# facebookresearch/mbrl-lib

Measured on AMD Instinct MI355X. Metric: candidate-steps/sec (pop×particles×horizon / plan) per CEM iter; plans/sec, higher is better.
Workload: dtype f32

## Files before the change

### mbrl-lib_amd/csrc/cem.hpp

```cpp
#pragma once
#include <type_traits>

#include "common.hpp"

namespace hipets {

struct CemDev {
    int n_env;
    int pop, H, A, D;
    int K;
    float alpha, one_minus_alpha;
    int return_mean, clipped, unbiased;
    const float* totals = nullptr;
    int P = 0;
    const int* elite_in = nullptr;
};

__device__ __forceinline__ float philox_trunc_normal(uint32_t idx_lo, uint32_t idx_hi, uint64_t seed, uint64_t stream) {
    for (uint32_t attempt = 0; attempt < 64; ++attempt) {
        const Philox4 r = philox4x32_10(idx_lo, idx_hi, attempt, (uint32_t)stream, (uint32_t)seed,
                                        (uint32_t)(seed >> 32) ^ (uint32_t)(stream >> 32) ^ 0x5EED5EEDu);
        float n0, n1, n2, n3;
        box_muller(r.x, r.y, n0, n1);
        if (fabsf(n0) <= 2.0f) return n0;
        if (fabsf(n1) <= 2.0f) return n1;
        box_muller(r.z, r.w, n2, n3);
        if (fabsf(n2) <= 2.0f) return n2;
        if (fabsf(n3) <= 2.0f) return n3;
    }
    return 0.0f;
}

__device__ __forceinline__ float philox_normal(uint32_t idx_lo, uint32_t idx_hi, uint64_t seed, uint64_t stream) {
    const Philox4 r = philox4x32_10(idx_lo, idx_hi, 0u, (uint32_t)stream, (uint32_t)seed,
                                    (uint32_t)(seed >> 32) ^ (uint32_t)(stream >> 32) ^ 0x5EED5EEDu);
    float n0, n1;
    box_muller(r.x, r.y, n0, n1);
    return n0;
}

__global__ void cem_sample_kernel(const CemDev p, const float* __restrict__ mu, const float* __restrict__ disp,
                                  const float* __restrict__ lower, const float* __restrict__ upper,
                                  const float* __restrict__ z_in, unsigned long long seed, unsigned long long stream,
                                  float* __restrict__ population) {
    const long long i = (long long)blockIdx.x * blockDim.x + threadIdx.x;
    if (i >= (long long)p.n_env * p.pop * p.D) return;
    const int d = (int)(i % p.D);
    const int env = (int)(i / ((long long)p.pop * p.D));
    const float m = mu[env * p.D + d], v = disp[env * p.D + d], lb = lower[d], ub = upper[d];
    float x;
    if (p.clipped) {
        const float z = z_in ? z_in[i] : philox_normal((uint32_t)i, (uint32_t)(i >> 32), seed, stream);
        x = m + v * z;
        x = x > lb ? x : lb;
        x = x < ub ? x : ub;
    } else {
        const float lbd = (m - lb) / 2.0f, ubd = (ub - m) / 2.0f;
        const float mv = fminf(lbd * lbd, ubd * ubd);
        const float cv = fminf(mv, v);
        const float z = z_in ? z_in[i] : philox_trunc_normal((uint32_t)i, (uint32_t)(i >> 32), seed, stream);
        x = z * sqrtf(cv) + m;
    }
    population[i] = x;
}

#ifndef HIPETS_REFIT_SKIP
#define HIPETS_REFIT_SKIP 0
#endif
constexpr int kRefitThreads = 1024;
constexpr int kMaxPop = 8192;
constexpr int kRefitScratchBytes = 12288;
constexpr int kSelectMaxK = 1024;
constexpr int kRankSortMax = 640;

__global__ __launch_bounds__(kRefitThreads) void cem_refit_kernel(const CemDev p, float* values, const float* population, float* mu,
                                                                 float* disp, float* best_value, float* best_solution,
                                                                 int* elite_idx_out) {
    extern __shared__ __attribute__((aligned(16))) char smem[];
    {
        const int env = blockIdx.y;
        values += (size_t)env * p.pop;
        if (p.totals && !(HIPETS_REFIT_SKIP & 1)) {
            const float* tot = p.totals + (size_t)env * p.pop * p.P;
            for (int i = threadIdx.x; i < p.pop; i += kRefitThreads) {
                float s = 0.f;
                for (int q0 = 0; q0 < p.P; q0 += 8) {
                    float tv[8];
#pragma unroll
                    for (int u = 0; u < 8; ++u) tv[u] = tot[(size_t)i * p.P + min(q0 + u, p.P - 1)];
#pragma unroll
                    for (int u = 0; u < 8; ++u)
                        if (q0 + u < p.P) s += tv[u];
                }
                values[i] = s / (float)p.P;
            }
        }
        population += (size_t)env * p.pop * p.D;
        mu += (size_t)env * p.D;
        disp += (size_t)env * p.D;
        best_value += env;
        best_solution += (size_t)env * p.D;
        if (elite_idx_out) elite_idx_out += (size_t)env * p.K;
    }
    const int* const elite_in = p.elite_in ? p.elite_in + (size_t)blockIdx.y * p.K : nullptr;
    int n2 = 1;
    while (n2 < p.pop) n2 <<= 1;
    float* key = reinterpret_cast<float*>(smem);
    int* idx = reinterpret_cast<int*>(smem + (size_t)n2 * 4);
    const int tid = threadIdx.x;
    for (int i = tid; i < n2; i += kRefitThreads) {
        float v = -INFINITY;
        if (i < p.pop) {
            v = values[i];
            if (v != v) { v = -1e-10f; values[i] = v; }
        }
        key[i] = v;
        idx[i] = i < p.pop ? i : 0x7FFFFFFF;
    }
    __syncthreads();
    if (elite_in) {
        auto in_range = [&](const int e) { return e < 0 ? 0 : (e >= p.pop ? p.pop - 1 : e); };
        const float top_key = key[in_range(elite_in[0])];
        __syncthreads();
        for (int k = tid; k < p.K; k += kRefitThreads) idx[k] = in_range(elite_in[k]);
        if (tid == 0) key[0] = top_key;
        __syncthreads();
    } else if (HIPETS_REFIT_SKIP & 2) {
    } else if (p.pop <= kRankSortMax) {
        for (int i = tid; i < p.pop; i += kRefitThreads) {
            const float ki = key[i];
            int rank = 0;
#pragma unroll 8
            for (int j = 0; j < i; ++j) rank += key[j] >= ki;
#pragma unroll 8
            for (int j = i + 1; j < p.pop; ++j) rank += key[j] > ki;
            idx[i] = rank;
        }
        __syncthreads();
        int* pos = reinterpret_cast<int*>(smem + (size_t)n2 * 8);
        for (int i = tid; i < p.pop; i += kRefitThreads) pos[idx[i]] = i;
        __syncthreads();
        float top_key = key[pos[0]];
        __syncthreads();
        for (int i = tid; i < p.pop; i += kRefitThreads) idx[i] = pos[i];
        if (tid == 0) key[0] = top_key;
        __syncthreads();
    } else if (p.K <= kSelectMaxK) {
        int* hist = reinterpret_cast<int*>(smem + (size_t)n2 * 8);
        int* ctl = hist + 256;
        int* elist = ctl + 8;
        float* ekey = reinterpret_cast<float*>(elist + kSelectMaxK);
        auto okey = [](float v) {
            const unsigned u = __float_as_uint(v + 0.0f);
            return (u & 0x80000000u) ? ~u : (u | 0x80000000u);
        };
        if (tid == 0) { ctl[0] = 0; ctl[1] = 0; ctl[2] = p.K; ctl[3] = 0; }
        for (int pass = 3; pass >= 0; --pass) {
            for (int b = tid; b < 256; b += kRefitThreads) hist[b] = 0;
            __syncthreads();
            const unsigned prefix = (unsigned)ctl[0], mask = (unsigned)ctl[1];
            for (int i = tid; i < p.pop; i += kRefitThreads) {
                const unsigned u = okey(key[i]);
                if ((u & mask) == prefix) atomicAdd(&hist[(u >> (8 * pass)) & 255u], 1);
            }
            __syncthreads();
            if (tid < 64) {
                const int h0 = hist[4 * tid], h1 = hist[4 * tid + 1], h2 = hist[4 * tid + 2], h3 = hist[4 * tid + 3];
                const int mine = h0 + h1 + h2 + h3;
                int above = mine;
#pragma unroll
                for (int d = 1; d < 64; d <<= 1) {
                    const int o = __shfl_down(above, d, 64);
                    if (tid + d < 64) above += o;
                }
                const int need = ctl[2];
                const int higher = above - mine;
                if (higher < need && need <= above) {
// ... 31 lines not shown
        if (tid < p.K) {
            my_id = elist[tid];
            my_key = ekey[tid];
            int rank = 0;
            for (int f = 0; f < p.K; ++f) {
                const float kf = ekey[f];
                rank += (kf > my_key) || (kf == my_key && elist[f] < my_id);
            }
            my_pos = rank;
        }
        __syncthreads();
        if (my_pos >= 0) idx[my_pos] = my_id;
        if (my_pos == 0) key[0] = my_key;
        __syncthreads();
    } else
    for (int k = 2; k <= n2; k <<= 1) {
        for (int j = k >> 1; j > 0; j >>= 1) {
            for (int i = tid; i < n2; i += kRefitThreads) {
                const int ixj = i ^ j;
                if (ixj > i) {
                    const float ka = key[i], kb = key[ixj];
                    const int ia = idx[i], ib = idx[ixj];
                    const bool a_first = (ka > kb) || (ka == kb && ia < ib);
                    const bool up = (i & k) == 0;
                    if (up ? !a_first : a_first) {
                        key[i] = kb; key[ixj] = ka;
                        idx[i] = ib; idx[ixj] = ia;
                    }
                }
            }
            __syncthreads();
        }
    }
    if (elite_idx_out && blockIdx.x == 0)
        for (int k = tid; k < p.K; k += kRefitThreads) elite_idx_out[k] = idx[k];

    const float top = key[0];
    const bool improved = blockIdx.x == 0 && top > best_value[0];
    const int top_i = idx[0];
    __syncthreads();

    double* red = reinterpret_cast<double*>(smem + (size_t)n2 * 8);
    const int nb = (int)gridDim.x, bx = (int)blockIdx.x;
    const int Dslice = (((p.D + nb - 1) / nb + 63) / 64) * 64;
    const int d_lo = bx * Dslice, d_hi = min(p.D, d_lo + Dslice);
    int parts = kRefitThreads / Dslice;
    parts = parts < 1 ? 1 : (parts > 8 ? 8 : parts);
    const int G = kRefitThreads / parts;
    const int part = tid / G, dloc = tid % G;
    const int nu = (p.K + parts - 1) / parts;
    auto sweep = [&](const int base, auto nu_tag, auto hold_tag) __attribute__((always_inline)) {
        constexpr int NU = decltype(nu_tag)::value;
        constexpr bool HOLD = decltype(hold_tag)::value;
        const int d = base + dloc;
        const bool live = d < d_hi && part < parts;
        float mu_old = 0.f, disp_old = 0.f;
        float xv[NU];
        double s = 0.0;
        if (live) {
            if (part == 0) { mu_old = mu[d]; disp_old = disp[d]; }
            for (int k0 = part; k0 < (HOLD ? part + 1 : p.K); k0 += parts * NU) {
#pragma unroll
                for (int u = 0; u < NU; ++u) xv[u] = population[(size_t)idx[min(k0 + u * parts, p.K - 1)] * p.D + d];
#pragma unroll
                for (int u = 0; u < NU; ++u)
                    if (k0 + u * parts < p.K) s += (double)xv[u];
            }
        }
        red[tid] = s;
        __syncthreads();
        double mean = 0.0;
        if (live) {
            for (int q = 0; q < parts; ++q) mean += red[q * G + dloc];
            mean /= (double)p.K;
        }
        __syncthreads();
        double ss = 0.0;
        if (live) {
            for (int k0 = part; k0 < (HOLD ? part + 1 : p.K); k0 += parts * NU) {
                if constexpr (!HOLD) {
#pragma unroll
                    for (int u = 0; u < NU; ++u) xv[u] = population[(size_t)idx[min(k0 + u * parts, p.K - 1)] * p.D + d];
                }
#pragma unroll
                for (int u = 0; u < NU; ++u)
                    if (k0 + u * parts < p.K) {
                        const double dv = (double)xv[u] - mean;
                        ss += dv * dv;
                    }
            }
        }
        red[tid] = ss;
        __syncthreads();
        if (live && part == 0) {
            double var = 0.0;
            for (int q = 0; q < parts; ++q) var += red[q * G + dloc];
            var /= (double)(p.unbiased ? (p.K - 1) : p.K);
            const float new_mu = (float)mean;
            const float new_disp = p.clipped ? (float)sqrt(var) : (float)var;
            mu[d] = p.alpha * mu_old + p.one_minus_alpha * new_mu;
            disp[d] = p.alpha * disp_old + p.one_minus_alpha * new_disp;
        }
        __syncthreads();
    };
    constexpr int kBestHold = 4;
    float best_row[kBestHold];
    const bool best_held = p.D <= kBestHold * kRefitThreads;
    if (improved && best_held) {
#pragma unroll
        for (int u = 0; u < kBestHold; ++u) best_row[u] = population[(size_t)top_i * p.D + min(tid + u * kRefitThreads, p.D - 1)];
    }
    for (int base = d_lo; base < ((HIPETS_REFIT_SKIP & 4) ? d_lo : d_hi); base += G) {
        using T = std::true_type;
        using F = std::false_type;
        if (nu <= 2) sweep(base, std::integral_constant<int, 2>{}, T{});
        else if (nu <= 4) sweep(base, std::integral_constant<int, 4>{}, T{});
        else if (nu <= 8) sweep(base, std::integral_constant<int, 8>{}, T{});
        else if (nu <= 16) sweep(base, std::integral_constant<int, 16>{}, T{});
        else sweep(base, std::integral_constant<int, 16>{}, F{});
    }
    if (improved) {
        if (best_held) {
#pragma unroll
            for (int u = 0; u < kBestHold; ++u)
                if (tid + u * kRefitThreads < p.D) best_solution[tid + u * kRefitThreads] = best_row[u];
        } else {
            for (int d = tid; d < p.D; d += kRefitThreads) best_solution[d] = population[(size_t)top_i * p.D + d];
        }
        if (tid == 0) best_value[0] = top;
    }
}

inline int refit_blocks(const int D) { return D <= 128 ? 1 : (D + 127) / 128 > 8 ? 8 : (D + 127) / 128; }

__global__ void cem_init_kernel(const CemDev p, const float* x0, const float* lower, const float* upper, float* mu,
                                float* disp, float* best_value) {
    const int i = blockIdx.x * blockDim.x + threadIdx.x;
    if (i < p.n_env * p.D) {
        const int d = i % p.D;
        mu[i] = x0[i];
        const float w = upper[d] - lower[d];
        disp[i] = p.clipped ? 1.0f : (w * w) / 16.0f;
    }
    if (i < p.n_env) best_value[i] = -INFINITY;
}

}
```

### mbrl-lib_amd/csrc/engine.hip

```cpp
#include <cstdarg>
#include <cstdio>
#include <cstring>

#include "engine.hpp"

namespace hipets {

thread_local std::string g_err;
thread_local int g_err_kind = HIPETS_ERR_NONE;

int fail(const char* fmt, ...) {
    char buf[1024];
    va_list ap;
    va_start(ap, fmt);
    vsnprintf(buf, sizeof(buf), fmt, ap);
    va_end(ap);
    g_err = buf;
    g_err_kind = HIPETS_ERR_INVALID_ARGUMENT;
    return 1;
}

int fail_kind(const int kind, const char* fmt, ...) {
    char buf[1024];
    va_list ap;
// ... 51 lines not shown

int hipets_create(int device, hipets_engine** out) {
    if (!out) return fail("null out pointer");
    *out = nullptr;
    int n = 0;
    hipError_t err = hipGetDeviceCount(&n);
    if (err != hipSuccess || n <= 0)
        return fail("no HIP device visible (%s) -- libhipets has no CPU fallback", hipGetErrorString(err));
    if (device < 0 || device >= n) return fail("device %d out of range (%d visible)", device, n);
    HCHECK(hipSetDevice(device));
    hipDeviceProp_t prop;
    HCHECK(hipGetDeviceProperties(&prop, device));
    if (std::string(prop.gcnArchName).rfind("gfx950", 0) != 0)
        return fail("device %d is %s; libhipets is built for gfx950 (MI355X) only", device, prop.gcnArchName);
    auto* e = new hipets_engine();
    e->device = device;
    e->num_cu = prop.multiProcessorCount > 0 ? prop.multiProcessorCount : 256;
    e->lds_max = prop.sharedMemPerBlockOptin > 0 ? (size_t)prop.sharedMemPerBlockOptin : (size_t)prop.sharedMemPerBlock;
    if (e->lds_max > 160 * 1024) e->lds_max = 160 * 1024;
    if (hipHostMalloc(reinterpret_cast<void**>(&e->error_flag), sizeof(int), hipHostMallocMapped) != hipSuccess) e->error_flag = nullptr;
    if (e->error_flag) *e->error_flag = 0;
    const char* np = std::getenv("HIPETS_NO_PERSISTENT");
    e->persistent_ok = e->error_flag != nullptr && !(np && np[0] == '1');
    if (e->census.ensure(2 * sizeof(int))) e->persistent_ok = false;
    *out = e;
    return 0;
}

void hipets_destroy(hipets_engine* e) {
    if (!e) return;
    (void)hipSetDevice(e->device);
    comm_release(e);
    for (DevBuf* b : {&e->w3pack, &e->wpack, &e->bpack, &e->layer_meta, &e->norm_mean, &e->norm_std, &e->min_lv, &e->max_lv, &e->no_delta, &e->members,
                      &e->s0, &e->state, &e->totals, &e->term, &e->exchange, &e->step_keys, &e->plan_keys, &e->mu, &e->disp, &e->population, &e->values,
                      &e->best_value, &e->best_solution, &e->past_action, &e->kept, &e->elite_idx, &e->keep_idx, &e->planet_w, &e->planet_b, &e->planet_member, &e->planet_ops, &e->shard_values, &e->gathered, &e->census, &e->train_slab, &e->train_partial})
        b->release();
    for (auto& ev : e->events) { (void)hipEventDestroy(ev.first); (void)hipEventDestroy(ev.second); }
    for (auto& ev : e->event_pool) { (void)hipEventDestroy(ev.first); (void)hipEventDestroy(ev.second); }
    if (e->error_flag) (void)hipHostFree(e->error_flag);
    if (e->last_done) (void)hipEventDestroy(e->last_done);
    for (auto& sl : e->stage) {
        if (sl.p) (void)hipHostFree(sl.p);
        if (sl.done) (void)hipEventDestroy(sl.done);
    }
    delete e;
}

int hipets_set_plan_mode(hipets_engine* e, int32_t mode) {
    if (!e) return fail("null engine");
    if (mode != HIPETS_MODE_FAST && mode != HIPETS_MODE_DEVICE) return fail("plan mode must be HIPETS_MODE_FAST or HIPETS_MODE_DEVICE");
    e->plan_mode = mode;
    return 0;
}

int hipets_set_persistent(hipets_engine* e, int32_t on) {
    if (!e) return fail("null engine");
    if (on && !e->error_flag) return fail("persistent DEVICE-mode launches need the host-mapped timeout flag, which could not be allocated");
    e->persistent_ok = on != 0;
    return 0;
}

int hipets_set_handover_timeout(hipets_engine* e, double seconds) {
    if (!e) return fail("null engine");
    if (!(seconds >= 0.0) || seconds > 60.0) return fail("hand-over timeout %g s outside [0, 60]", seconds);
    e->poll_ticks = (long long)(seconds * 1.0e8);
    return 0;
}
// ... 52 lines not shown
```

### mbrl-lib_amd/csrc/engine.hpp

```cpp
#pragma once
#include <hip/hip_runtime.h>

#include <cstdlib>
#include <string>
#include <utility>
#include <vector>

#include "../../include/hipets.h"
#include "planet_types.hpp"
#include "rollout_types.hpp"

namespace hipets {

extern thread_local std::string g_err;
extern thread_local int g_err_kind;

}

#pragma GCC visibility push(hidden)

namespace hipets {

int fail(const char* fmt, ...);
int fail_kind(int kind, const char* fmt, ...);
// ... 26 lines not shown
    T* as() const { return reinterpret_cast<T*>(p); }
};

}

#pragma GCC visibility pop

struct hipets_engine {
    using DevBuf = hipets::DevBuf;
    int device = 0;
    int num_cu = 256;
    size_t lds_max = 160 * 1024;
    bool has_model = false;
    hipets::ModelDev md{};
    int ensemble_size = 0;
    DevBuf w3pack;
    DevBuf wpack, bpack, layer_meta, norm_mean, norm_std, min_lv, max_lv, no_delta, members;
    DevBuf s0, state, totals, term;
    DevBuf exchange, step_keys, plan_keys;
    struct HostStage { void* p = nullptr; size_t cap = 0; hipEvent_t done = nullptr; bool used = false; };
    HostStage stage[4];
    int stage_next = 0;
    uint32_t tag_base = 0;
    uint64_t plan_keys_seed = 0, plan_keys_first = 0;
    int plan_keys_count = 0, plan_keys_H = 0;
    int* error_flag = nullptr;
    bool persistent_ok = true;
    long long poll_ticks = 20000000ll;
    DevBuf census;
    hipStream_t last_stream = nullptr;
    bool last_stream_set = false;
    hipEvent_t last_done = nullptr;
    DevBuf mu, disp, population, values, best_value, best_solution, past_action, kept, elite_idx, keep_idx;
    void* comm = nullptr;
    int comm_rank = 0, comm_world = 1;
    DevBuf shard_values, gathered;
    bool has_planet = false;
    bool planet_static = false;
    hipets::PlanetDev pd{};
    DevBuf planet_w, planet_b, planet_member, planet_ops;
    int plan_mode = HIPETS_MODE_FAST;
    bool has_trace = false;
    hipets_plan_trace trace{};
    bool timing = false;
    int timing_stride = 1;
    unsigned long long launch_counter = 0;
    std::vector<std::pair<hipEvent_t, hipEvent_t>> events;
    std::vector<std::pair<hipEvent_t, hipEvent_t>> event_pool;
    DevBuf train_slab, train_partial;
};

#pragma GCC visibility push(hidden)

namespace hipets {


int stage_h2d(hipets_engine* e, void* dst, const void* src, size_t bytes, hipStream_t st);

int enter_stream(hipets_engine* e, hipStream_t st);
struct StreamScope {
    hipets_engine* e;
    hipStream_t st;
    ~StreamScope();
};
#define ENTER_STREAM(e, st)                \
    if (enter_stream((e), (st))) return 1; \
// ... 39 lines not shown
```

### mbrl-lib_amd/csrc/plan.hip

```cpp
#include <algorithm>
#include <cmath>
#include <vector>

#include "engine.hpp"
#include "lds_optin.hpp"
#include "optim.hpp"

using namespace hipets;

namespace {

int launch_mppi_sample(int n_env, int pop, int H, int A, float beta, const float* mean, const float* past_action, const float* lower, const float* upper,
                       const float* z, uint64_t seed, uint64_t stream_id, float* population, hipStream_t st) {
    const long long npop = (long long)n_env * pop;
    const long long D = (long long)H * A;
    if (D <= kMppiSampleMaxD) {
        const int G = mppi_sample_group(npop, (int)D);
        hipLaunchKernelGGL(mppi_sample_staged_kernel, dim3((unsigned)((npop + G - 1) / G)), dim3(kMppiSampleThreads), (size_t)G * D * 4, st, n_env, pop, H, A, G, beta,
                           mean, past_action, lower, upper, z, (unsigned long long)seed, (unsigned long long)stream_id, population);
    } else {
        const long long n = npop * A;
        hipLaunchKernelGGL(mppi_sample_kernel, dim3((unsigned)((n + 255) / 256)), dim3(256), 0, st, n_env, pop, H, A, beta, mean, past_action, lower, upper, z,
                           (unsigned long long)seed, (unsigned long long)stream_id, population);
    }
// ... 152 lines not shown
    o.kind = PlanObjective::PLANET;
    o.latent0 = latent0;
    o.belief0 = belief0;
    return o;
}

int check_plan(const hipets_engine* e, const PlanObjective& obj, bool args, int A, int n_env, int P) {
    const bool planet = obj.is_planet();
    if (planet && !(e && e->has_planet)) return fail("engine has no PlaNet model (call hipets_planet_set_model)");
    if (!planet && !(e && e->has_model)) return fail("engine has no model (call hipets_set_model)");
    if (!args || (planet ? !(obj.latent0 && obj.belief0) : !obj.s0)) return fail("null argument");
    if (planet && A != e->pd.action) return fail("act_dim %d != model action_size %d", A, e->pd.action);
    if (!planet && A != e->md.act_dim) return fail("act_dim %d != model act_dim %d", A, e->md.act_dim);
    if (n_env < 1 || n_env > 4096) return fail("n_env %d outside [1, 4096]", n_env);
    if (planet && P < 1) return fail("bad pop/horizon/particles");
    return 0;
}

int launch_cem_refit(const CemDev& c, float* values, const float* population, float* mu, float* disp, float* best_value, float* best_solution,
                     int* elite_idx, hipStream_t st) {
    int n2 = 1;
    while (n2 < c.pop) n2 <<= 1;
    hipLaunchKernelGGL(cem_refit_kernel, dim3(refit_blocks(c.D), c.n_env), dim3(kRefitThreads), (size_t)n2 * 8 + kRefitScratchBytes, st, c, values,
                       population, mu, disp, best_value, best_solution, elite_idx);
    HCHECK(hipGetLastError());
    return 0;
}

struct PlanLoop {
    int n_env, H, P, iters;
    uint64_t first_stream, stream_stride, rollout_stream;
    const float* population;
    float* returns;
};
template <class Prologue, class Rows, class Sample, class Refit>
int run_plan(hipets_engine* e, const PlanObjective& obj, const PlanLoop& pl, uint64_t seed, void* stream, Prologue prologue, Rows rows, Sample sample,
             Refit refit) {
    hipets_rollout_opts ro{};
    ro.mode = e->plan_mode;
    ro.seed = obj.rollout_seed(e, seed);
    ro.n_env = pl.n_env;
    const bool carry_on = obj.is_sharded();
    LocalErr le;
    le.note(prologue(ro.seed));
    for (int i = 0; i < pl.iters && (carry_on || le.ok()); ++i) {
        const uint64_t sid = (pl.first_stream + (uint64_t)i) * pl.stream_stride;
        if (le.ok()) le.note(sample(i, sid));
        ro.stream_id = sid + pl.rollout_stream;
        if (obj.evaluate(e, pl.population, rows(i), pl.H, pl.P, &ro, pl.returns, stream, le)) return 1;
        if (le.ok()) le.note(refit(i));
    }
    return le.report();
}

int plan_cem_impl(hipets_engine* e, const hipets_cem_params* p, int32_t n_env, const float* x0, const float* lower, const float* upper,
                  const PlanObjective& obj, int32_t P, uint64_t seed, uint64_t plan_id, float* out, void* stream) {
    if (check_cem(p) || check_plan(e, obj, x0 && lower && upper && out, p->act_dim, n_env, P)) return 1;
    if (obj.is_sharded() && check_shards(e, p->population_size, P)) return 1;
    hipStream_t st = reinterpret_cast<hipStream_t>(stream);
    HCHECK(hipSetDevice(e->device));
    ENTER_STREAM(e, st);
    const CemDev c = make_cem(p, n_env);
    const size_t nd = (size_t)n_env * c.D, npop = (size_t)n_env * c.pop;
    if (e->mu.ensure(nd * 4) || e->disp.ensure(nd * 4) || e->best_solution.ensure(nd * 4) || e->best_value.ensure((size_t)n_env * 4 + 16) ||
        e->population.ensure(npop * c.D * 4) || e->values.ensure(npop * 4) || obj.reserve_shards(e, c.pop))
        return 1;
    const int iters = p->num_iterations;
    const PlanLoop pl{n_env, c.H, P, iters, plan_id * (uint64_t)iters, 1, 0, e->population.as<float>(), nullptr};
    auto prologue = [&](uint64_t rollout_seed) -> int {
        if (obj.clear_padding(e, c.pop, st)) return 1;
        hipLaunchKernelGGL(cem_init_kernel, dim3((unsigned)((nd + 255) / 256)), dim3(256), 0, st, c, x0, lower, upper, e->mu.as<float>(),
                           e->disp.as<float>(), e->best_value.as<float>());
        HCHECK(hipGetLastError());
        HCHECK(hipMemsetAsync(e->best_solution.p, 0, nd * 4, st));
        return obj.is_planet() ? 0 : plan_prologue(e, obj.s0, n_env, c.H, iters, rollout_seed, pl.first_stream, st);
    };
    auto sample = [&](int, uint64_t sid) -> int {
        const long long n = (long long)npop * c.D;
        hipLaunchKernelGGL(cem_sample_kernel, dim3((unsigned)((n + 255) / 256)), dim3(256), 0, st, c, e->mu.as<float>(), e->disp.as<float>(),
                           lower, upper, (const float*)nullptr, (unsigned long long)seed, (unsigned long long)sid, e->population.as<float>());
        HCHECK(hipGetLastError());
        return 0;
    };
    auto refit = [&](int i) -> int {
        int* eidx = (e->has_trace && e->trace.elite_idx) ? e->trace.elite_idx + (size_t)i * n_env * c.K : nullptr;
        CemDev cr = c;
        obj.refit_from_totals(e, &cr, P);
        if (launch_cem_refit(cr, e->values.as<float>(), e->population.as<float>(), e->mu.as<float>(), e->disp.as<float>(), e->best_value.as<float>(),
                             e->best_solution.as<float>(), eidx, st))
            return 1;
        return trace_iter(e, i, (int)npop, (size_t)c.D, e->population.as<float>(), e->values.as<float>(), e->mu.as<float>(), e->disp.as<float>(), st, n_env);
    };
    if (run_plan(e, obj, pl, seed, stream, prologue, [&](int) { return (int)npop; }, sample, refit)) return 1;
    HCHECK(hipMemcpyAsync(out, p->return_mean_elites ? e->mu.p : e->best_solution.p, nd * 4, hipMemcpyDeviceToDevice, st));
    return 0;
}

int plan_mppi_impl(hipets_engine* e, int32_t pop, int32_t H, int32_t A, int32_t num_iterations, double gamma, double beta, int32_t n_env,
                   float* mean, const float* lower, const float* upper, const PlanObjective& obj, int32_t P, uint64_t seed, uint64_t plan_id,
                   void* stream) {
    if (check_plan(e, obj, mean && lower && upper, A, n_env, P)) return 1;
    if (pop < 1 || pop > 12000) return fail("population_size %d outside [1, 12000]", pop);
    if (H < 1 || num_iterations < 0) return fail("bad horizon/num_iterations");
    if (obj.is_sharded() && check_shards(e, pop, P)) return 1;
    hipStream_t st = reinterpret_cast<hipStream_t>(stream);
    HCHECK(hipSetDevice(e->device));
    ENTER_STREAM(e, st);
    const size_t nd = (size_t)H * A, npop = (size_t)n_env * pop;
    if (e->mu.ensure(n_env * nd * 4) || e->past_action.ensure((size_t)n_env * A * 4) || e->population.ensure(npop * nd * 4) ||
        e->values.ensure(npop * 4) || obj.reserve_shards(e, pop))
        return 1;
    const PlanLoop pl{n_env, H, P, num_iterations, plan_id * (uint64_t)num_iterations, 1, 0, e->population.as<float>(), e->values.as<float>()};
    auto prologue = [&](uint64_t rollout_seed) -> int {
        if (obj.clear_padding(e, pop, st)) return 1;
        HCHECK(hipMemcpyAsync(e->mu.p, mean, n_env * nd * 4, hipMemcpyDeviceToDevice, st));
        hipLaunchKernelGGL(mppi_shift_kernel, dim3((unsigned)((n_env * nd + 255) / 256)), dim3(256), 0, st, n_env, H, A, e->mu.as<float>(), mean,
                           e->past_action.as<float>());
        HCHECK(hipGetLastError());
        return obj.is_planet() ? 0 : plan_prologue(e, obj.s0, n_env, H, num_iterations, rollout_seed, pl.first_stream, st);
    };
    auto sample = [&](int, uint64_t sid) -> int {
        return launch_mppi_sample(n_env, pop, H, A, (float)beta, mean, e->past_action.as<float>(), lower, upper, nullptr, seed, sid,
                                  e->population.as<float>(), st);
    };
    auto update = [&](int k) -> int {
        if (launch_mppi_update(e, n_env, pop, (int)nd, (float)gamma, e->values.as<float>(), e->population.as<float>(), mean, st)) return 1;
        return trace_iter(e, k, (int)npop, nd, e->population.as<float>(), e->values.as<float>(), mean, nullptr, st, n_env);
    };
// ... 286 lines not shown
```

Before: 290.8 million.

## Fuse CEM refit with next-iteration sampling into one boundary kernel per iteration

Splits the CEM refit into reusable selection and sweep helpers. It adds a fused prologue kernel that does init plus the first sample, and a boundary kernel that refits and then draws the next population from the new mean and dispersion in the same launch, writing into a double-buffered population. This removes separate sample, init and memset launches and their global round trips between CEM iterations. The rank-sort path is also split across several threads per element using float4 LDS reads and partial-rank reduction. The cost is more complex multi-block coordination, LDS staging of totals, and a risk of ordering or RNG-stream mismatches.

```diff
diff --git a/mbrl-lib_amd/csrc/cem.hpp b/mbrl-lib_amd/csrc/cem.hpp
--- a/mbrl-lib_amd/csrc/cem.hpp
+++ b/mbrl-lib_amd/csrc/cem.hpp
@@ -39,17 +39,11 @@
     return n0;
 }
 
-__global__ void cem_sample_kernel(const CemDev p, const float* __restrict__ mu, const float* __restrict__ disp,
-                                  const float* __restrict__ lower, const float* __restrict__ upper,
-                                  const float* __restrict__ z_in, unsigned long long seed, unsigned long long stream,
-                                  float* __restrict__ population) {
-    const long long i = (long long)blockIdx.x * blockDim.x + threadIdx.x;
-    if (i >= (long long)p.n_env * p.pop * p.D) return;
-    const int d = (int)(i % p.D);
-    const int env = (int)(i / ((long long)p.pop * p.D));
-    const float m = mu[env * p.D + d], v = disp[env * p.D + d], lb = lower[d], ub = upper[d];
+__device__ __forceinline__ float cem_draw(const int clipped, const float m, const float v, const float lb, const float ub,
+                                          const float* __restrict__ z_in, const long long i, const unsigned long long seed,
+                                          const unsigned long long stream) {
     float x;
-    if (p.clipped) {
+    if (clipped) {
         const float z = z_in ? z_in[i] : philox_normal((uint32_t)i, (uint32_t)(i >> 32), seed, stream);
         x = m + v * z;
         x = x > lb ? x : lb;
@@ -61,7 +55,18 @@
         const float z = z_in ? z_in[i] : philox_trunc_normal((uint32_t)i, (uint32_t)(i >> 32), seed, stream);
         x = z * sqrtf(cv) + m;
     }
-    population[i] = x;
+    return x;
+}
+
+__global__ void cem_sample_kernel(const CemDev p, const float* __restrict__ mu, const float* __restrict__ disp,
+                                  const float* __restrict__ lower, const float* __restrict__ upper,
+                                  const float* __restrict__ z_in, unsigned long long seed, unsigned long long stream,
+                                  float* __restrict__ population) {
+    const long long i = (long long)blockIdx.x * blockDim.x + threadIdx.x;
+    if (i >= (long long)p.n_env * p.pop * p.D) return;
+    const int d = (int)(i % p.D);
+    const int env = (int)(i / ((long long)p.pop * p.D));
+    population[i] = cem_draw(p.clipped, mu[env * p.D + d], disp[env * p.D + d], lower[d], upper[d], z_in, i, seed, stream);
 }
 
 #ifndef HIPETS_REFIT_SKIP
@@ -73,51 +78,17 @@
 constexpr int kSelectMaxK = 1024;
 constexpr int kRankSortMax = 640;
 
-__global__ __launch_bounds__(kRefitThreads) void cem_refit_kernel(const CemDev p, float* values, const float* population, float* mu,
-                                                                 float* disp, float* best_value, float* best_solution,
-                                                                 int* elite_idx_out) {
-    extern __shared__ __attribute__((aligned(16))) char smem[];
-    {
-        const int env = blockIdx.y;
-        values += (size_t)env * p.pop;
-        if (p.totals && !(HIPETS_REFIT_SKIP & 1)) {
-            const float* tot = p.totals + (size_t)env * p.pop * p.P;
-            for (int i = threadIdx.x; i < p.pop; i += kRefitThreads) {
-                float s = 0.f;
-                for (int q0 = 0; q0 < p.P; q0 += 8) {
-                    float tv[8];
-#pragma unroll
-                    for (int u = 0; u < 8; ++u) tv[u] = tot[(size_t)i * p.P + min(q0 + u, p.P - 1)];
-#pragma unroll
-                    for (int u = 0; u < 8; ++u)
-                        if (q0 + u < p.P) s += tv[u];
-                }
-                values[i] = s / (float)p.P;
-            }
-        }
-        population += (size_t)env * p.pop * p.D;
-        mu += (size_t)env * p.D;
-        disp += (size_t)env * p.D;
-        best_value += env;
-        best_solution += (size_t)env * p.D;
-        if (elite_idx_out) elite_idx_out += (size_t)env * p.K;
-    }
-    const int* const elite_in = p.elite_in ? p.elite_in + (size_t)blockIdx.y * p.K : nullptr;
-    int n2 = 1;
-    while (n2 < p.pop) n2 <<= 1;
+__host__ __device__ inline int refit_blocks(const int D) { return D <= 128 ? 1 : (D + 127) / 128 > 8 ? 8 : (D + 127) / 128; }
+__host__ __device__ inline int refit_slice(const int D, const int nb) { return (((D + nb - 1) / nb + 63) / 64) * 64; }
+__host__ __device__ inline int refit_parts(const int Dslice) {
+    const int parts = kRefitThreads / Dslice;
+    return parts < 1 ? 1 : (parts > 8 ? 8 : parts);
+}
+
+__device__ __forceinline__ void cem_select(const CemDev& p, char* smem, const int n2, const int* elite_in) {
     float* key = reinterpret_cast<float*>(smem);
     int* idx = reinterpret_cast<int*>(smem + (size_t)n2 * 4);
     const int tid = threadIdx.x;
-    for (int i = tid; i < n2; i += kRefitThreads) {
-        float v = -INFINITY;
-        if (i < p.pop) {
-            v = values[i];
-            if (v != v) { v = -1e-10f; values[i] = v; }
-        }
-        key[i] = v;
-        idx[i] = i < p.pop ? i : 0x7FFFFFFF;
-    }
-    __syncthreads();
     if (elite_in) {
         auto in_range = [&](const int e) { return e < 0 ? 0 : (e >= p.pop ? p.pop - 1 : e); };
         const float top_key = key[in_range(elite_in[0])];
@@ -127,22 +98,49 @@
         __syncthreads();
     } else if (HIPETS_REFIT_SKIP & 2) {
     } else if (p.pop <= kRankSortMax) {
-        for (int i = tid; i < p.pop; i += kRefitThreads) {
-            const float ki = key[i];
-            int rank = 0;
+        const int share = p.pop <= 256 ? 4 : (p.pop <= 512 ? 2 : 1);
+        const int E = kRefitThreads / share;
+        const int i = tid % E;
+        const int sub = __builtin_amdgcn_readfirstlane(tid / E);
+        const int w_lo = __builtin_amdgcn_readfirstlane(i);
+        const int nq = (p.pop + 3) >> 2;
+        const int q_lo = sub * nq / share, q_hi = (sub + 1) * nq / share;
+        const float ki = key[i < p.pop ? i : p.pop - 1];
+        const float4* key4 = reinterpret_cast<const float4*>(key);
+        const int qA = w_lo >> 2, qB = qA + 16, qF = p.pop >> 2;
+        auto mixed = [&](const int q) {
+            const float4 kq = key4[q];
+            const int j = 4 * q;
+            auto one = [&](const float kj, const int jj) { return (int)(jj < p.pop && (jj < i ? kj >= ki : kj > ki)); };
+            return one(kq.x, j) + one(kq.y, j + 1) + one(kq.z, j + 2) + one(kq.w, j + 3);
+        };
+        int rank = 0;
+        const int a_hi = min(q_hi, qA), b_lo = max(q_lo, qA), b_hi = min(q_hi, qB), c_lo = max(q_lo, qB), c_hi = min(q_hi, qF);
 #pragma unroll 8
-            for (int j = 0; j < i; ++j) rank += key[j] >= ki;
+        for (int q = q_lo; q < a_hi; ++q) {
+            const float4 kq = key4[q];
+            rank += (int)(kq.x >= ki) + (int)(kq.y >= ki) + (int)(kq.z >= ki) + (int)(kq.w >= ki);
+        }
+        for (int q = b_lo; q < b_hi; ++q) rank += mixed(q);
 #pragma unroll 8
-            for (int j = i + 1; j < p.pop; ++j) rank += key[j] > ki;
-            idx[i] = rank;
-        }
-        __syncthreads();
+        for (int q = c_lo; q < c_hi; ++q) {
+            const float4 kq = key4[q];
+            rank += (int)(kq.x > ki) + (int)(kq.y > ki) + (int)(kq.z > ki) + (int)(kq.w > ki);
+        }
+        if (qF < nq && qF >= c_lo && qF < q_hi) rank += mixed(qF);
         int* pos = reinterpret_cast<int*>(smem + (size_t)n2 * 8);
-        for (int i = tid; i < p.pop; i += kRefitThreads) pos[idx[i]] = i;
+        int* partial = pos + kRefitThreads;
+        partial[tid] = rank;
+        __syncthreads();
+        for (int e = tid; e < p.pop; e += kRefitThreads) {
+            int r = 0;
+            for (int s = 0; s < share; ++s) r += partial[s * E + e];
+            pos[r] = e;
+        }
         __syncthreads();
         float top_key = key[pos[0]];
         __syncthreads();
-        for (int i = tid; i < p.pop; i += kRefitThreads) idx[i] = pos[i];
+        for (int e = tid; e < p.pop; e += kRefitThreads) idx[e] = pos[e];
         if (tid == 0) key[0] = top_key;
         __syncthreads();
     } else if (p.K <= kSelectMaxK) {
@@ -240,20 +238,13 @@
             __syncthreads();
         }
     }
-    if (elite_idx_out && blockIdx.x == 0)
-        for (int k = tid; k < p.K; k += kRefitThreads) elite_idx_out[k] = idx[k];
-
-    const float top = key[0];
-    const bool improved = blockIdx.x == 0 && top > best_value[0];
-    const int top_i = idx[0];
-    __syncthreads();
-
+}
+
+__device__ __forceinline__ void cem_sweeps(const CemDev& p, char* smem, const int n2, const float* population, float* mu, float* disp,
+                                           const int d_lo, const int d_hi, const int parts, float* fresh, const int fresh_w) {
+    const int* idx = reinterpret_cast<const int*>(smem + (size_t)n2 * 4);
     double* red = reinterpret_cast<double*>(smem + (size_t)n2 * 8);
-    const int nb = (int)gridDim.x, bx = (int)blockIdx.x;
-    const int Dslice = (((p.D + nb - 1) / nb + 63) / 64) * 64;
-    const int d_lo = bx * Dslice, d_hi = min(p.D, d_lo + Dslice);
-    int parts = kRefitThreads / Dslice;
-    parts = parts < 1 ? 1 : (parts > 8 ? 8 : parts);
+    const int tid = threadIdx.x;
     const int G = kRefitThreads / parts;
     const int part = tid / G, dloc = tid % G;
     const int nu = (p.K + parts - 1) / parts;
@@ -306,18 +297,14 @@
             var /= (double)(p.unbiased ? (p.K - 1) : p.K);
             const float new_mu = (float)mean;
             const float new_disp = p.clipped ? (float)sqrt(var) : (float)var;
-            mu[d] = p.alpha * mu_old + p.one_minus_alpha * new_mu;
-            disp[d] = p.alpha * disp_old + p.one_minus_alpha * new_disp;
+            const float m = p.alpha * mu_old + p.one_minus_alpha * new_mu;
+            const float v = p.alpha * disp_old + p.one_minus_alpha * new_disp;
+            mu[d] = m;
+            disp[d] = v;
+            if (fresh) { fresh[d - d_lo] = m; fresh[fresh_w + d - d_lo] = v; }
         }
         __syncthreads();
     };
-    constexpr int kBestHold = 4;
-    float best_row[kBestHold];
-    const bool best_held = p.D <= kBestHold * kRefitThreads;
-    if (improved && best_held) {
-#pragma unroll
-        for (int u = 0; u < kBestHold; ++u) best_row[u] = population[(size_t)top_i * p.D + min(tid + u * kRefitThreads, p.D - 1)];
-    }
     for (int base = d_lo; base < ((HIPETS_REFIT_SKIP & 4) ? d_lo : d_hi); base += G) {
         using T = std::true_type;
         using F = std::false_type;
@@ -327,6 +314,73 @@
         else if (nu <= 16) sweep(base, std::integral_constant<int, 16>{}, T{});
         else sweep(base, std::integral_constant<int, 16>{}, F{});
     }
+}
+
+__global__ __launch_bounds__(kRefitThreads) void cem_refit_kernel(const CemDev p, float* values, const float* population, float* mu,
+                                                                 float* disp, float* best_value, float* best_solution,
+                                                                 int* elite_idx_out) {
+    extern __shared__ __attribute__((aligned(16))) char smem[];
+    {
+        const int env = blockIdx.y;
+        values += (size_t)env * p.pop;
+        if (p.totals && !(HIPETS_REFIT_SKIP & 1)) {
+            const float* tot = p.totals + (size_t)env * p.pop * p.P;
+            for (int i = threadIdx.x; i < p.pop; i += kRefitThreads) {
+                float s = 0.f;
+                for (int q0 = 0; q0 < p.P; q0 += 8) {
+                    float tv[8];
+#pragma unroll
+                    for (int u = 0; u < 8; ++u) tv[u] = tot[(size_t)i * p.P + min(q0 + u, p.P - 1)];
+#pragma unroll
+                    for (int u = 0; u < 8; ++u)
+                        if (q0 + u < p.P) s += tv[u];
+                }
+                values[i] = s / (float)p.P;
+            }
+        }
+        population += (size_t)env * p.pop * p.D;
+        mu += (size_t)env * p.D;
+        disp += (size_t)env * p.D;
+        best_value += env;
+        best_solution += (size_t)env * p.D;
+        if (elite_idx_out) elite_idx_out += (size_t)env * p.K;
+    }
+    const int* const elite_in = p.elite_in ? p.elite_in + (size_t)blockIdx.y * p.K : nullptr;
+    int n2 = 1;
+    while (n2 < p.pop) n2 <<= 1;
+    float* key = reinterpret_cast<float*>(smem);
+    int* idx = reinterpret_cast<int*>(smem + (size_t)n2 * 4);
+    const int tid = threadIdx.x;
+    for (int i = tid; i < n2; i += kRefitThreads) {
+        float v = -INFINITY;
+        if (i < p.pop) {
+            v = values[i];
+            if (v != v) { v = -1e-10f; values[i] = v; }
+        }
+        key[i] = v;
+        idx[i] = i < p.pop ? i : 0x7FFFFFFF;
+    }
+    __syncthreads();
+    cem_select(p, smem, n2, elite_in);
+    if (elite_idx_out && blockIdx.x == 0)
+        for (int k = tid; k < p.K; k += kRefitThreads) elite_idx_out[k] = idx[k];
+
+    const float top = key[0];
+    const bool improved = blockIdx.x == 0 && top > best_value[0];
+    const int top_i = idx[0];
+    __syncthreads();
+
+    const int nb = (int)gridDim.x, bx = (int)blockIdx.x;
+    const int Dslice = refit_slice(p.D, nb);
+    const int d_lo = bx * Dslice, d_hi = min(p.D, d_lo + Dslice);
+    constexpr int kBestHold = 4;
+    float best_row[kBestHold];
+    const bool best_held = p.D <= kBestHold * kRefitThreads;
+    if (improved && best_held) {
+#pragma unroll
+        for (int u = 0; u < kBestHold; ++u) best_row[u] = population[(size_t)top_i * p.D + min(tid + u * kRefitThreads, p.D - 1)];
+    }
+    cem_sweeps(p, smem, n2, population, mu, disp, d_lo, d_hi, refit_parts(Dslice), nullptr, 0);
     if (improved) {
         if (best_held) {
 #pragma unroll
@@ -339,7 +393,136 @@
     }
 }
 
-inline int refit_blocks(const int D) { return D <= 128 ? 1 : (D + 127) / 128 > 8 ? 8 : (D + 127) / 128; }
+constexpr int kPlanSliceMax = 16;
+__host__ __device__ inline int plan_slice(const int D) { return D <= 256 ? 4 : (D <= 512 ? 8 : kPlanSliceMax); }
+inline int plan_blocks(const int D) { return (D + plan_slice(D) - 1) / plan_slice(D); }
+
+struct CemNext {
+    const float* lower;
+    const float* upper;
+    unsigned long long seed, stream;
+    float* next_population;
+    float* out;
+    int stage_rows;
+};
+
+template <class M, class V>
+__device__ __forceinline__ void cem_draw_slice(const CemDev& p, const int env, const int d_lo, const int d_hi, const float* __restrict__ lower,
+                                               const float* __restrict__ upper, const unsigned long long seed, const unsigned long long stream,
+                                               float* __restrict__ population, M m_of, V v_of) {
+    const int w = d_hi - d_lo;
+    for (int t = threadIdx.x; t < p.pop * w; t += kRefitThreads) {
+        const int c = t / w, d = d_lo + t % w;
+        const long long i = ((long long)env * p.pop + c) * p.D + d;
+        population[i] = cem_draw(p.clipped, m_of(d), v_of(d), lower[d], upper[d], nullptr, i, seed, stream);
+    }
+}
+
+__global__ __launch_bounds__(kRefitThreads) void cem_prologue_kernel(const CemDev p, const float* __restrict__ x0, const float* __restrict__ lower,
+                                                                    const float* __restrict__ upper, float* __restrict__ mu,
+                                                                    float* __restrict__ disp, float* __restrict__ best_value,
+                                                                    float* __restrict__ best_solution, const unsigned long long seed,
+                                                                    const unsigned long long stream, float* __restrict__ population) {
+    const int env = blockIdx.y, W = plan_slice(p.D);
+    const int d_lo = blockIdx.x * W, d_hi = min(p.D, d_lo + W);
+    auto disp0 = [&](const int d) {
+        const float w = upper[d] - lower[d];
+        return p.clipped ? 1.0f : (w * w) / 16.0f;
+    };
+    const int d = d_lo + (int)threadIdx.x;
+    if (d < d_hi) {
+        mu[env * p.D + d] = x0[env * p.D + d];
+        disp[env * p.D + d] = disp0(d);
+        best_solution[env * p.D + d] = 0.0f;
+    }
+    if (blockIdx.x == 0 && threadIdx.x == 0) best_value[env] = -INFINITY;
+    cem_draw_slice(p, env, d_lo, d_hi, lower, upper, seed, stream, population, [&](const int dd) { return x0[env * p.D + dd]; }, disp0);
+}
+
+__global__ __launch_bounds__(kRefitThreads) void cem_boundary_kernel(const CemDev p, float* values, const float* population, float* mu,
+                                                                    float* disp, float* best_value, float* best_solution,
+                                                                    int* elite_idx_out, const CemNext nx) {
+    extern __shared__ __attribute__((aligned(16))) char smem[];
+    const int env = blockIdx.y, tid = threadIdx.x;
+    const bool first = blockIdx.x == 0;
+    values += (size_t)env * p.pop;
+    population += (size_t)env * p.pop * p.D;
+    mu += (size_t)env * p.D;
+    disp += (size_t)env * p.D;
+    best_value += env;
+    best_solution += (size_t)env * p.D;
+    if (elite_idx_out) elite_idx_out += (size_t)env * p.K;
+    int n2 = 1;
+    while (n2 < p.pop) n2 <<= 1;
+    float* key = reinterpret_cast<float*>(smem);
+    int* idx = reinterpret_cast<int*>(smem + (size_t)n2 * 4);
+    auto filtered = [](const float v) { return v != v ? -1e-10f : v; };
+    for (int i = tid; i < n2; i += kRefitThreads) {
+        idx[i] = i < p.pop ? i : 0x7FFFFFFF;
+        if (i >= p.pop) key[i] = -INFINITY;
+    }
+    if (!p.totals) {
+        for (int i = tid; i < p.pop; i += kRefitThreads) {
+            const float raw = values[i], v = filtered(raw);
+            key[i] = v;
+            if (first && raw != raw) values[i] = v;
+        }
+    } else {
+        const float* tot = p.totals + (size_t)env * p.pop * p.P;
+        auto store = [&](const int i, const float s) {
+            const float v = filtered(s / (float)p.P);
+            key[i] = v;
+            if (first) values[i] = v;
+        };
+        if (nx.stage_rows > 0) {
+            float* stage = reinterpret_cast<float*>(smem + (size_t)n2 * 8 + kRefitScratchBytes);
+            for (int c0 = 0; c0 < p.pop; c0 += nx.stage_rows) {
+                const int rows = min(nx.stage_rows, p.pop - c0);
+                if (c0) __syncthreads();
+                for (int t = tid; t < rows * p.P; t += kRefitThreads) stage[t] = tot[(size_t)c0 * p.P + t];
+                __syncthreads();
+                for (int r = tid; r < rows; r += kRefitThreads) {
+                    float s = 0.f;
+                    for (int q = 0; q < p.P; ++q) s += stage[r * p.P + q];
+                    store(c0 + r, s);
+                }
+            }
+        } else {
+            for (int i = tid; i < p.pop; i += kRefitThreads) {
+                float s = 0.f;
+                for (int q = 0; q < p.P; ++q) s += tot[(size_t)i * p.P + q];
+                store(i, s);
+            }
+        }
+    }
+    __syncthreads();
+    cem_select(p, smem, n2, nullptr);
+    if (elite_idx_out && first)
+        for (int k = tid; k < p.K; k += kRefitThreads) elite_idx_out[k] = idx[k];
+
+    const float top = key[0];
+    const bool improved = first && top > best_value[0];
+    const int top_i = idx[0];
+    __syncthreads();
+
+    const int W = plan_slice(p.D);
+    const int d_lo = blockIdx.x * W, d_hi = min(p.D, d_lo + W);
+    float* fresh = reinterpret_cast<float*>(smem + (size_t)n2 * 8 + kRefitThreads * sizeof(double));
+    cem_sweeps(p, smem, n2, population, mu, disp, d_lo, d_hi, refit_parts(refit_slice(p.D, refit_blocks(p.D))), fresh, kPlanSliceMax);
+    if (improved) {
+        for (int d = tid; d < p.D; d += kRefitThreads) best_solution[d] = population[(size_t)top_i * p.D + d];
+        if (tid == 0) best_value[0] = top;
+    }
+    if (nx.next_population) {
+        cem_draw_slice(p, env, d_lo, d_hi, nx.lower, nx.upper, nx.seed, nx.stream, nx.next_population,
+                       [&](const int d) { return fresh[d - d_lo]; }, [&](const int d) { return fresh[kPlanSliceMax + d - d_lo]; });
+    } else if (p.return_mean) {
+        if (d_lo + tid < d_hi) nx.out[(size_t)env * p.D + d_lo + tid] = fresh[tid];
+    } else if (first) {
+        for (int d = tid; d < p.D; d += kRefitThreads)
+            nx.out[(size_t)env * p.D + d] = improved ? population[(size_t)top_i * p.D + d] : best_solution[d];
+    }
+}
 
 __global__ void cem_init_kernel(const CemDev p, const float* x0, const float* lower, const float* upper, float* mu,
                                 float* disp, float* best_value) {
diff --git a/mbrl-lib_amd/csrc/engine.hip b/mbrl-lib_amd/csrc/engine.hip
--- a/mbrl-lib_amd/csrc/engine.hip
+++ b/mbrl-lib_amd/csrc/engine.hip
@@ -107,7 +107,7 @@
     (void)hipSetDevice(e->device);
     comm_release(e);
     for (DevBuf* b : {&e->w3pack, &e->wpack, &e->bpack, &e->layer_meta, &e->norm_mean, &e->norm_std, &e->min_lv, &e->max_lv, &e->no_delta, &e->members,
-                      &e->s0, &e->state, &e->totals, &e->term, &e->exchange, &e->step_keys, &e->plan_keys, &e->mu, &e->disp, &e->population, &e->values,
+                      &e->s0, &e->state, &e->totals, &e->term, &e->exchange, &e->step_keys, &e->plan_keys, &e->mu, &e->disp, &e->population, &e->population_alt, &e->values,
                       &e->best_value, &e->best_solution, &e->past_action, &e->kept, &e->elite_idx, &e->keep_idx, &e->planet_w, &e->planet_b, &e->planet_member, &e->planet_ops, &e->shard_values, &e->gathered, &e->census, &e->train_slab, &e->train_partial})
         b->release();
     for (auto& ev : e->events) { (void)hipEventDestroy(ev.first); (void)hipEventDestroy(ev.second); }
diff --git a/mbrl-lib_amd/csrc/engine.hpp b/mbrl-lib_amd/csrc/engine.hpp
--- a/mbrl-lib_amd/csrc/engine.hpp
+++ b/mbrl-lib_amd/csrc/engine.hpp
@@ -82,6 +82,7 @@
     bool last_stream_set = false;
     hipEvent_t last_done = nullptr;
     DevBuf mu, disp, population, values, best_value, best_solution, past_action, kept, elite_idx, keep_idx;
+    DevBuf population_alt;
     void* comm = nullptr;
     int comm_rank = 0, comm_world = 1;
     DevBuf shard_values, gathered;
diff --git a/mbrl-lib_amd/csrc/plan.hip b/mbrl-lib_amd/csrc/plan.hip
--- a/mbrl-lib_amd/csrc/plan.hip
+++ b/mbrl-lib_amd/csrc/plan.hip
@@ -208,6 +208,7 @@
     uint64_t first_stream, stream_stride, rollout_stream;
     const float* population;
     float* returns;
+    const float* population_alt = nullptr;
 };
 template <class Prologue, class Rows, class Sample, class Refit>
 int run_plan(hipets_engine* e, const PlanObjective& obj, const PlanLoop& pl, uint64_t seed, void* stream, Prologue prologue, Rows rows, Sample sample,
@@ -223,7 +224,8 @@
         const uint64_t sid = (pl.first_stream + (uint64_t)i) * pl.stream_stride;
         if (le.ok()) le.note(sample(i, sid));
         ro.stream_id = sid + pl.rollout_stream;
-        if (obj.evaluate(e, pl.population, rows(i), pl.H, pl.P, &ro, pl.returns, stream, le)) return 1;
+        const float* population = (pl.population_alt && (i & 1)) ? pl.population_alt : pl.population;
+        if (obj.evaluate(e, population, rows(i), pl.H, pl.P, &ro, pl.returns, stream, le)) return 1;
         if (le.ok()) le.note(refit(i));
     }
     return le.report();
@@ -239,37 +241,39 @@
     const CemDev c = make_cem(p, n_env);
     const size_t nd = (size_t)n_env * c.D, npop = (size_t)n_env * c.pop;
     if (e->mu.ensure(nd * 4) || e->disp.ensure(nd * 4) || e->best_solution.ensure(nd * 4) || e->best_value.ensure((size_t)n_env * 4 + 16) ||
-        e->population.ensure(npop * c.D * 4) || e->values.ensure(npop * 4) || obj.reserve_shards(e, c.pop))
+        e->population.ensure(npop * c.D * 4) || e->population_alt.ensure(npop * c.D * 4) || e->values.ensure(npop * 4) || obj.reserve_shards(e, c.pop))
         return 1;
     const int iters = p->num_iterations;
-    const PlanLoop pl{n_env, c.H, P, iters, plan_id * (uint64_t)iters, 1, 0, e->population.as<float>(), nullptr};
+    float* const popbuf[2] = {e->population.as<float>(), e->population_alt.as<float>()};
+    const PlanLoop pl{n_env, c.H, P, iters, plan_id * (uint64_t)iters, 1, 0, popbuf[0], nullptr, popbuf[1]};
+    const dim3 grid(plan_blocks(c.D), n_env);
     auto prologue = [&](uint64_t rollout_seed) -> int {
         if (obj.clear_padding(e, c.pop, st)) return 1;
-        hipLaunchKernelGGL(cem_init_kernel, dim3((unsigned)((nd + 255) / 256)), dim3(256), 0, st, c, x0, lower, upper, e->mu.as<float>(),
-                           e->disp.as<float>(), e->best_value.as<float>());
+        hipLaunchKernelGGL(cem_prologue_kernel, grid, dim3(kRefitThreads), 0, st, c, x0, lower, upper, e->mu.as<float>(), e->disp.as<float>(),
+                           e->best_value.as<float>(), e->best_solution.as<float>(), (unsigned long long)seed, (unsigned long long)pl.first_stream,
+                           popbuf[0]);
         HCHECK(hipGetLastError());
-        HCHECK(hipMemsetAsync(e->best_solution.p, 0, nd * 4, st));
+        if (iters < 1) HCHECK(hipMemcpyAsync(out, p->return_mean_elites ? e->mu.p : e->best_solution.p, nd * 4, hipMemcpyDeviceToDevice, st));
         return obj.is_planet() ? 0 : plan_prologue(e, obj.s0, n_env, c.H, iters, rollout_seed, pl.first_stream, st);
     };
-    auto sample = [&](int, uint64_t sid) -> int {
-        const long long n = (long long)npop * c.D;
-        hipLaunchKernelGGL(cem_sample_kernel, dim3((unsigned)((n + 255) / 256)), dim3(256), 0, st, c, e->mu.as<float>(), e->disp.as<float>(),
-                           lower, upper, (const float*)nullptr, (unsigned long long)seed, (unsigned long long)sid, e->population.as<float>());
-        HCHECK(hipGetLastError());
-        return 0;
-    };
-    auto refit = [&](int i) -> int {
+    auto boundary = [&](int i) -> int {
         int* eidx = (e->has_trace && e->trace.elite_idx) ? e->trace.elite_idx + (size_t)i * n_env * c.K : nullptr;
         CemDev cr = c;
         obj.refit_from_totals(e, &cr, P);
-        if (launch_cem_refit(cr, e->values.as<float>(), e->population.as<float>(), e->mu.as<float>(), e->disp.as<float>(), e->best_value.as<float>(),
-                             e->best_solution.as<float>(), eidx, st))
-            return 1;
-        return trace_iter(e, i, (int)npop, (size_t)c.D, e->population.as<float>(), e->values.as<float>(), e->mu.as<float>(), e->disp.as<float>(), st, n_env);
-    };
-    if (run_plan(e, obj, pl, seed, stream, prologue, [&](int) { return (int)npop; }, sample, refit)) return 1;
-    HCHECK(hipMemcpyAsync(out, p->return_mean_elites ? e->mu.p : e->best_solution.p, nd * 4, hipMemcpyDeviceToDevice, st));
-    return 0;
+        const bool last = i == iters - 1;
+        int n2 = 1;
+        while (n2 < c.pop) n2 <<= 1;
+        const size_t lds = (size_t)n2 * 8 + kRefitScratchBytes;
+        const size_t row = (size_t)std::max(cr.P, 1) * 4, room = lds < 65536 ? (65536 - lds) / row : 0;
+        const int stage_rows = (cr.totals && room >= (size_t)std::min(c.pop, 64)) ? (int)std::min<size_t>(room, (size_t)c.pop) : 0;
+        const CemNext nx{lower, upper, (unsigned long long)seed, (unsigned long long)(pl.first_stream + (uint64_t)i + 1), last ? nullptr : popbuf[(i + 1) & 1],
+                         out, stage_rows};
+        hipLaunchKernelGGL(cem_boundary_kernel, grid, dim3(kRefitThreads), lds + (size_t)stage_rows * row, st, cr, e->values.as<float>(), popbuf[i & 1],
+                           e->mu.as<float>(), e->disp.as<float>(), e->best_value.as<float>(), e->best_solution.as<float>(), eidx, nx);
+        HCHECK(hipGetLastError());
+        return trace_iter(e, i, (int)npop, (size_t)c.D, popbuf[i & 1], e->values.as<float>(), e->mu.as<float>(), e->disp.as<float>(), st, n_env);
+    };
+    return run_plan(e, obj, pl, seed, stream, prologue, [&](int) { return (int)npop; }, [](int, uint64_t) { return 0; }, boundary);
 }
 
 int plan_mppi_impl(hipets_engine* e, int32_t pop, int32_t H, int32_t A, int32_t num_iterations, double gamma, double beta, int32_t n_env,
diff --git a/profiles/plan_boundary_probe.py b/profiles/plan_boundary_probe.py
--- /dev/null
+++ b/profiles/plan_boundary_probe.py
@@ -0,0 +1,134 @@
+import argparse
+import csv
+import glob
+import json
+import os
+import shutil
+import statistics
+import subprocess
+import sys
+import tempfile
+
+ROOT = os.path.dirname(os.path.dirname(os.path.abspath(__file__)))
+BENCH = [sys.executable, os.path.join(ROOT, "bench.py"), "--gpus", "1", "--no-extras", "--no-cpu-baseline"]
+PLAN_MARKERS = ("cem_prologue_kernel", "cem_init_kernel")
+
+
+def drive(which, plans):
+    sys.path[:0] = [ROOT, os.path.join(ROOT, "mbrl-lib_amd")]
+    import numpy as np
+    import torch
+
+    import bench
+    import hipets
+    from hipets.planning import _BoundObjective
+
+    dev = torch.device("cuda:0")
+    eng = hipets.get_engine(dev)
+    if which == "cfg1":
+        spec = bench.synthetic_spec(dev, obs=4, act=1, ensemble=5, reward="cartpole", termination="cartpole")
+        fn = hipets.make_eval_fn(spec, 5, engine=eng, seed=0)
+        H, act = 15, 1
+        opt = hipets.CEMOptimizer(5, 0.1, 100, [[-1.0] * act] * H, [[1.0] * act] * H, 0.1, dev, return_mean_elites=True, seed=0)
+        obj = _BoundObjective(fn, np.zeros(4, np.float32))
+    else:
+        spec = bench.synthetic_planet_spec(dev)
+        eng.planet_set_model(spec)
+        fn = hipets.make_eval_fn(spec, 1, engine=eng, seed=0)
+        fn.set_state(torch.zeros(1, 30), torch.zeros(1, 200))
+        H, act = 12, 6
+        opt = hipets.CEMOptimizer(10, 0.1, 1000, [[-1.0] * act] * H, [[1.0] * act] * H, 0.0, dev, return_mean_elites=True, clipped_normal=True, seed=1)
+        obj = _BoundObjective(fn, np.zeros((3, 64, 64), np.float32))
+    x0 = torch.zeros(H, act, device=dev)
+    for _ in range(plans):
+        out = opt.optimize(obj, x0=x0)
+    torch.cuda.synchronize()
+    assert torch.isfinite(out).all()
+
+
+def child(cmd, env, limit, log):
+    with open(log, "w") as f:
+        rc = subprocess.run(["timeout", "-k", "10", str(limit)] + cmd, env=env, stdout=f, stderr=subprocess.STDOUT, cwd=ROOT).returncode
+    if rc != 0:
+        tail = "".join(open(log, errors="replace").readlines()[-15:])
+        raise SystemExit(f"[plan_boundary_probe] step failed (exit {rc}): {' '.join(cmd)}\n{tail}")
+
+
+def trace(cmd, env, workdir, tag):
+    d = os.path.join(workdir, tag)
+    child(["rocprofv3", "--kernel-trace", "--stats", "--output-format", "csv", "-d", d, "-o", "t", "--"] + cmd, env, 240, os.path.join(workdir, tag + ".log"))
+    files = glob.glob(os.path.join(d, "**", "*kernel_stats.csv"), recursive=True)
+    if not files:
+        raise SystemExit(f"[plan_boundary_probe] no kernel_stats.csv under {d}")
+    rows = [(r["Name"], int(r["Calls"]), float(r["TotalDurationNs"])) for f in files for r in csv.DictReader(open(f))]
+    plans = sum(c for n, c, _ in rows if any(m in n for m in PLAN_MARKERS))
+    rollout = [(n, c, t) for n, c, t in rows if "rollout_kernel" in n]
+    other = [(n, c, t) for n, c, t in rows if "rollout_kernel" not in n]
+    return {"plans": plans, "launches_per_plan": sum(c for _, c, _ in rows) / plans,
+            "non_rollout_us_per_plan": sum(t for _, _, t in other) / plans / 1e3,
+            "rollout_us_per_plan": sum(t for _, _, t in rollout) / plans / 1e3,
+            "kernels": {n.split("(")[0][-60:]: {"calls_per_plan": c / plans, "us_each": t / c / 1e3} for n, c, t in rows}}
+
+
+def headline(env, workdir, tag, steps, warmup):
+    log = os.path.join(workdir, tag + ".log")
+    child(BENCH + ["--steps", str(steps), "--warmup", str(warmup)], env, 240, log)
+    for line in reversed(open(log, errors="replace").readlines()):
+        if line.startswith("{"):
+            r = json.loads(line)
+            return r["ms_per_step"], (r.get("roofline") or {}).get("avg_launch_ms")
+    raise SystemExit(f"[plan_boundary_probe] no result line in {log}")
+
+
+def main():
+    ap = argparse.ArgumentParser()
+    ap.add_argument("--parent-lib")
+    ap.add_argument("--runs", type=int, default=5)
+    ap.add_argument("--steps", type=int, default=200)
+    ap.add_argument("--warmup", type=int, default=20)
+    ap.add_argument("--out", default=os.path.join(ROOT, "profiles", "plan_boundary.json"))
+    ap.add_argument("--also", action="append", default=[], metavar="NAME=LIB", help="trace a further build of the library (a kernel variant) as well")
+    ap.add_argument("--drive", choices=["cfg1", "planet"])
+    ap.add_argument("--plans", type=int, default=30)
+    args = ap.parse_args()
+    if args.drive:
+        return drive(args.drive, args.plans)
+    if not args.parent_lib or not os.path.exists(args.parent_lib):
+        raise SystemExit("--parent-lib: a libhipets.so built from the parent commit")
+    envs = {"parent": dict(os.environ, HIPETS_LIB=os.path.abspath(args.parent_lib)), "new": {k: v for k, v in os.environ.items() if k != "HIPETS_LIB"}}
+    for extra in args.also:
+        name, lib = extra.split("=", 1)
+        envs[name] = dict(os.environ, HIPETS_LIB=os.path.abspath(lib))
+    workdir = tempfile.mkdtemp(prefix="plan_boundary_")
+    me = [sys.executable, os.path.abspath(__file__)]
+    res = {"command": f"bench.py {' '.join(BENCH[2:])} --steps {args.steps} --warmup {args.warmup} (trace runs: --steps 20 --warmup 3)", "trace": {}, "headline": {}}
+    for side, env in envs.items():
+        res["trace"][side] = {"cfg2": trace(BENCH + ["--steps", "20", "--warmup", "3"], env, workdir, f"trace_cfg2_{side}"),
+                              "cfg1": trace(me + ["--drive", "cfg1"], env, workdir, f"trace_cfg1_{side}"),
+                              "planet": trace(me + ["--drive", "planet"], env, workdir, f"trace_planet_{side}")}
+    runs = {"parent": [], "new": []}
+    for i in range(args.runs):
+        for side in ("parent", "new"):
+            runs[side].append(headline(envs[side], workdir, f"bench_{side}_{i}", args.steps, args.warmup))
+            print(f"[plan_boundary_probe] run {i} {side}: ms_per_step {runs[side][-1][0]:.4f}, rollout avg_launch_ms {runs[side][-1][1]}", flush=True)
+    for side, rr in runs.items():
+        ms, launch = [r[0] for r in rr], [r[1] for r in rr if r[1] is not None]
+        res["headline"][side] = {"ms_per_step": ms, "median": statistics.median(ms), "spread": max(ms) - min(ms),
+                                 "rollout_avg_launch_ms": launch, "rollout_avg_launch_ms_median": statistics.median(launch) if launch else None}
+    h = res["headline"]
+    gain = h["parent"]["median"] - h["new"]["median"]
+    res["headline"]["gain_ms"] = gain
+    res["headline"]["gain_over_larger_spread"] = gain / max(h["parent"]["spread"], h["new"]["spread"], 1e-9)
+    res["acceptance"] = {
+        "headline_gain_exceeds_three_spreads": gain > 3 * max(h["parent"]["spread"], h["new"]["spread"]),
+        "non_rollout_time_dropped": {w: res["trace"]["new"][w]["non_rollout_us_per_plan"] < res["trace"]["parent"][w]["non_rollout_us_per_plan"]
+                                     for w in ("cfg2", "cfg1", "planet")}}
+    with open(args.out, "w") as f:
+        json.dump(res, f, indent=1)
+    shutil.rmtree(workdir, ignore_errors=True)
+    print(json.dumps({k: res[k] for k in ("headline", "acceptance")}, indent=1))
+    print({s: {w: (round(t["launches_per_plan"], 2), round(t["non_rollout_us_per_plan"], 1)) for w, t in res["trace"][s].items()} for s in res["trace"]})
+
+
+if __name__ == "__main__":
+    main()
```

After: 291.6 million, median of 6. About the same (+0.3%).
